# tengdj/lsbm

Hardware: AMD Instinct MI355X
Metric: CRC32C GiB/s over device-resident 4 KiB SSTable blocks (1 GPU); % HBM peak (higher is better)
Workload: dtype u8; 1 GPU; 1048576 x 4096 B device-resident blocks per GPU, batched crc32c::Value; blocks_per_gpu=1048576, block_bytes=4096, stride=4096, parallelism=1 independent shards, no data-path collective

## Files before the change

include/lsbm_crc32c.h:

```cpp
#ifndef LSBM_CRC32C_H_
#define LSBM_CRC32C_H_

#include <stddef.h>
#include <stdint.h>

#ifdef __cplusplus
extern "C" {
#endif

#define LSBM_OK 0
#define LSBM_ERR_INVALID (-1)
#define LSBM_ERR_NO_DEVICE (-2)
#define LSBM_ERR_HIP (-3)
#define LSBM_ERR_NOMEM (-4)
#define LSBM_ERR_CORRUPTION (-5)

#define LSBM_CRC32C_MASKED 0x1u

#define LSBM_CRC32C_MASK_DELTA 0xa282ead8u
#define LSBM_BLOCK_TRAILER_SIZE 5

uint32_t lsbm_crc32c_extend(uint32_t init_crc, const char* data, size_t n);
uint32_t lsbm_crc32c_value(const char* data, size_t n);
uint32_t lsbm_crc32c_mask(uint32_t crc);
uint32_t lsbm_crc32c_unmask(uint32_t masked_crc);

int lsbm_crc32c_init(int device);
int lsbm_crc32c_shutdown(void);
const char* lsbm_crc32c_version(void);
const char* lsbm_crc32c_last_error(void);

int lsbm_crc32c_fixed_dev(const void* d_base, uint64_t stride, uint64_t len, uint64_t n_blocks,
                          const uint32_t* d_init, uint32_t* d_out, uint32_t flags, void* stream);

int lsbm_crc32c_batch_dev(const void* d_base, const uint64_t* d_offsets, uint64_t n_blocks,
                          const uint32_t* d_init, uint32_t* d_out, uint32_t flags, void* stream);

int lsbm_crc32c_extents_dev(const void* d_base, const uint64_t* d_extents, uint64_t n_blocks,
// ... 16 lines not shown
int lsbm_log_crcs_dev(const uint8_t* d_log, uint64_t log_bytes, const uint64_t* d_headers,
                      uint64_t n_records, uint32_t* d_masked, uint32_t* d_nbad, void* stream);
int lsbm_log_verify_dev(const uint8_t* d_log, uint64_t log_bytes, const uint64_t* d_headers,
                        uint64_t n_records, uint8_t* d_ok, uint32_t* d_nbad, void* stream);

int lsbm_crc32c_batch_host(int device, const void* h_base, const uint64_t* h_offsets,
                           uint64_t n_blocks, const uint32_t* h_init, uint32_t* h_out,
                           uint32_t flags);

int lsbm_crc32c_batch_host_multi(const int* devices, int n_devices, const void* h_base,
                                 const uint64_t* h_offsets, uint64_t n_blocks,
                                 const uint32_t* h_init, uint32_t* h_out, uint32_t flags);

int lsbm_gather_dev(const void* d_src, const uint64_t* d_src_off, const uint64_t* d_len, uint64_t n,
                    void* d_dst, const uint64_t* d_dst_off, void* stream);

int lsbm_fill_splitmix64_dev(void* d_buf, uint64_t nbytes, uint64_t seed, void* stream);
int lsbm_stream_read_dev(const void* d_buf, uint64_t nbytes, uint32_t* d_sink, void* stream);

int lsbm_test_fail_host_pipeline(int chunks);
int lsbm_test_ragged_kernel(int which);

int lsbm_test_fixed_queue(int on);
int lsbm_test_sst_pieces(int on);

int lsbm_host_threads(void);

int lsbm_host_register(const void* p, uint64_t n);
int lsbm_host_unregister(const void* p);
unsigned long long lsbm_host_registered_bytes(void);
int lsbm_device_numa_node(int device);
int lsbm_test_pci_numa_node(const char* sysfs_root, const char* bus_id);
int lsbm_test_parse_cpulist(const char* list, int* cpus, int cap);
int lsbm_test_cgroup_quota(const char* cgroup_root);
int lsbm_test_pool_overlap(int callers, int jobs, int pieces, int piece_us, double* seconds);
int lsbm_test_cgroup_quota_of(const char* cgroup_root, const char* proc_cgroup);
int lsbm_test_pool_helpers(int pieces, int piece_us, int max_helpers);
int lsbm_test_locked_ranges(void);
long lsbm_test_locks_taken(void);
int lsbm_test_session_count(int device);
unsigned long long lsbm_test_pinned_bytes(int device);
int lsbm_test_pool_stress(int callers, int jobs, int max_pieces);
int lsbm_test_host_pinned(const void* p, size_t n);
int lsbm_test_zero_copy_max_mb(int mb);
int lsbm_test_host_copy(void* dst, const void* src, size_t n, int parallel);

// ... 6 lines not shown
```

lsbm_amd/_lib.py:

```python
import ctypes
import os

_HERE = os.path.dirname(os.path.abspath(__file__))
LIB_PATH = os.path.join(_HERE, "liblsbm_crc32c.so")
LIB_PATH = os.environ.get("LSBM_LIB_PATH") or LIB_PATH

LSBM_OK = 0
LSBM_ERR_INVALID = -1
LSBM_ERR_NO_DEVICE = -2
LSBM_ERR_HIP = -3
LSBM_ERR_NOMEM = -4
LSBM_ERR_CORRUPTION = -5
LSBM_CRC32C_MASKED = 0x1
LSBM_CRC32C_MASK_DELTA = 0xA282EAD8
LSBM_BLOCK_TRAILER_SIZE = 5

_u32, _u64, _int, _vp, _sz = (ctypes.c_uint32, ctypes.c_uint64, ctypes.c_int,
                              ctypes.c_void_p, ctypes.c_size_t)
SIGNATURES = {
    "lsbm_crc32c_extend": (_u32, [_u32, _vp, _sz]),
    "lsbm_crc32c_value": (_u32, [_vp, _sz]),
    "lsbm_crc32c_mask": (_u32, [_u32]),
    "lsbm_crc32c_unmask": (_u32, [_u32]),
    "lsbm_crc32c_init": (_int, [_int]),
    "lsbm_crc32c_shutdown": (_int, []),
    "lsbm_crc32c_version": (ctypes.c_char_p, []),
    "lsbm_crc32c_last_error": (ctypes.c_char_p, []),
    "lsbm_crc32c_fixed_dev": (_int, [_vp, _u64, _u64, _u64, _vp, _vp, _u32, _vp]),
    "lsbm_crc32c_batch_dev": (_int, [_vp, _vp, _u64, _vp, _vp, _u32, _vp]),
    "lsbm_crc32c_extents_dev": (_int, [_vp, _vp, _u64, _vp, _vp, _u32, _vp]),
    "lsbm_crc32c_verify_dev": (_int, [_vp, _vp, _u64, _vp, _vp, _vp, _vp, _u32, _vp]),
    "lsbm_sst_seal_dev": (_int, [_vp, _u64, _vp, _vp, _u64, _vp, _vp]),
    "lsbm_sst_verify_dev": (_int, [_vp, _u64, _vp, _u64, _vp, _vp, _vp]),
    "lsbm_sst_trailer_crcs_dev": (_int, [_vp, _u64, _vp, _vp, _u64, _vp, _vp, _vp]),
    "lsbm_log_seal_dev": (_int, [_vp, _u64, _vp, _u64, _vp, _vp, _vp]),
    "lsbm_log_verify_dev": (_int, [_vp, _u64, _vp, _u64, _vp, _vp, _vp]),
    "lsbm_log_crcs_dev": (_int, [_vp, _u64, _vp, _u64, _vp, _vp, _vp]),
    "lsbm_crc32c_batch_host": (_int, [_int, _vp, _vp, _u64, _vp, _vp, _u32]),
    "lsbm_crc32c_batch_host_multi": (_int, [_vp, _int, _vp, _vp, _u64, _vp, _vp, _u32]),
    "lsbm_gather_dev": (_int, [_vp, _vp, _vp, _u64, _vp, _vp, _vp]),
    "lsbm_fill_splitmix64_dev": (_int, [_vp, _u64, _u64, _vp]),
    "lsbm_stream_read_dev": (_int, [_vp, _u64, _vp, _vp]),
    "lsbm_test_fail_host_pipeline": (_int, [_int]),
    "lsbm_test_ragged_kernel": (_int, [_int]),
    "lsbm_test_fixed_queue": (_int, [_int]),
    "lsbm_test_sst_pieces": (_int, [_int]),
    "lsbm_host_threads": (_int, []),
    "lsbm_host_register": (_int, [ctypes.c_void_p, ctypes.c_uint64]),
    "lsbm_host_unregister": (_int, [ctypes.c_void_p]),
    "lsbm_host_registered_bytes": (ctypes.c_ulonglong, []),
    "lsbm_device_numa_node": (_int, [_int]),
    "lsbm_test_pci_numa_node": (_int, [ctypes.c_char_p, ctypes.c_char_p]),
    "lsbm_test_parse_cpulist": (_int, [ctypes.c_char_p, _vp, _int]),
    "lsbm_test_cgroup_quota": (_int, [ctypes.c_char_p]),
    "lsbm_test_cgroup_quota_of": (_int, [ctypes.c_char_p, ctypes.c_char_p]),
    "lsbm_test_pool_helpers": (_int, [_int, _int, _int]),
    "lsbm_test_locked_ranges": (_int, []),
    "lsbm_test_locks_taken": (ctypes.c_long, []),
    "lsbm_test_session_count": (_int, [_int]),
    "lsbm_test_pinned_bytes": (ctypes.c_ulonglong, [_int]),
    "lsbm_test_pool_overlap": (_int, [_int, _int, _int, _int, _vp]),
    "lsbm_test_host_pinned": (_int, [_vp, _sz]),
    "lsbm_test_host_copy": (_int, [_vp, _vp, _sz, _int]),
    "lsbm_test_pool_stress": (_int, [_int, _int, _int]),
    "lsbm_test_zero_copy_max_mb": (_int, [_int]),
    "lsbm_bloom_hash": (_u32, [_vp, _sz, _u32]),
    "lsbm_bloom_filter_bytes": (_u64, [_u64, _int]),
    "lsbm_bloom_k": (_u32, [_int]),
# ... 68 lines not shown
```

lsbm_amd/csrc/crc32c_engine.cc:

```cpp
#include <hip/hip_runtime_api.h>
#include <stdint.h>
#include <stdio.h>
#include <stdlib.h>
#include <string.h>

#include <algorithm>
#include <atomic>
#include <mutex>
#include <new>
#include <string>
#include <thread>
#include <vector>

#include "../../include/lsbm_crc32c.h"
#include "crc32c_types.h"
#include "engine_internal.h"
#include "gf2.h"
#include "host_numa.h"
#include "host_session.h"

namespace lsbm {

hipError_t launch_fixed(const uint8_t* base, uint64_t stride, uint32_t rows, uint64_t n_blocks,
                        const uint32_t* init, uint32_t* out, uint32_t flags, uint32_t k_value,
                        const DevConsts* dc, int grid, hipStream_t stream,
                        uint32_t* heads);
hipError_t launch_ragged(const RaggedArgs& a, int grid, hipStream_t stream);
bool ragged_uses_stream(const RaggedArgs& a);
int set_ragged_policy(int p);
hipError_t launch_range_bounds(const RaggedArgs& a, uint64_t P, uint32_t* bounds, int grid,
                               hipStream_t stream);
hipError_t launch_trailer_scatter(uint8_t* file, uint64_t limit, const uint64_t* handles, const uint8_t* types,
                                  const uint32_t* crcs, uint64_t n, int grid, hipStream_t stream);
hipError_t launch_fill(uint8_t* buf, uint64_t nbytes, uint64_t seed, int grid, hipStream_t stream);
hipError_t launch_gather(const uint8_t* src, const uint64_t* src_off, const uint64_t* len, uint64_t n,
                         uint8_t* dst, const uint64_t* dst_off, int grid, hipStream_t stream);
hipError_t launch_stream_read(const void* buf, uint64_t nbytes, uint32_t* sink, int grid,
                              hipStream_t stream);

namespace {

thread_local char t_last_error[256] = "";

int fail_hip(hipError_t e, const char* what) {
  snprintf(t_last_error, sizeof(t_last_error), "%s: %s", what, hipGetErrorString(e));
  return LSBM_ERR_HIP;
}
int fail(int code, const char* what) {
  snprintf(t_last_error, sizeof(t_last_error), "%s", what);
  return code;
}

constexpr int kMaxDevices = 64;

struct DeviceState {
  std::mutex mu;
  std::atomic<bool> ready{false};
  int status = LSBM_ERR_NO_DEVICE;
  DevConsts* d_consts = nullptr;
  int num_cus = 0;
};
DeviceState g_dev[kMaxDevices];

void build_consts(DevConsts* c) {
  gf2::byte_tables(gf2::byte_pow(kRowBytes), c->row_byte);
  {
    uint32_t tmp[1024];
    gf2::byte_tables(gf2::byte_pow(1), tmp);
    memcpy(c->t0, tmp, sizeof(c->t0));
  }
  gf2::Mat p = gf2::byte_pow(1);
  for (int k = 0; k < 64; k++) {
    gf2::nibble_tables(p, c->pow_nib[k]);
    p = gf2::mul(p, p);
  }
  const gf2::Mat inv1 = gf2::byte_pow(-1), fwd1 = gf2::byte_pow(1);
  {
    gf2::Mat m = gf2::identity();
    for (int z = 0; z < 128; z++, m = gf2::mul(inv1, m)) gf2::nibble_tables(m, c->neg_nib[z]);
  }
  gf2::nibble_tables(gf2::byte_pow(-4), c->neg4_nib);
  for (int li = 0; li < 8; li++) gf2::nibble_tables(gf2::byte_pow(116 - 16 * li), c->fin_nib[li]);
  memset(c->lds_image, 0, sizeof(c->lds_image));
#ifdef LSBM_LDS16
  {
// ... 68 lines not shown
  DevConsts* h = new (std::nothrow) DevConsts;
  if (!h) {
    st->status = fail(LSBM_ERR_NOMEM, "host alloc");
    hipSetDevice(prev);
    return;
  }
  build_consts(h);
  DevConsts* d = nullptr;
  e = hipMalloc(&d, sizeof(DevConsts));
  if (e == hipSuccess) e = hipMemcpy(d, h, sizeof(DevConsts), hipMemcpyHostToDevice);
  delete h;
  if (e != hipSuccess) {
    st->status = fail_hip(e, "device tables");
    if (d) hipFree(d);
    hipSetDevice(prev);
    return;
  }
  hipMemPool_t pool = nullptr;
  if (hipDeviceGetDefaultMemPool(&pool, dev) == hipSuccess && pool) {
    uint64_t keep = ~0ull;
    (void)hipMemPoolSetAttribute(pool, hipMemPoolAttrReleaseThreshold, &keep);
  }
  (void)hipGetLastError();
  st->d_consts = d;
  st->num_cus = cus;
  st->status = LSBM_OK;
  hipSetDevice(prev);
}

int ensure_device(int dev, DeviceState** out) {
  if (dev < 0 || dev >= kMaxDevices) return fail(LSBM_ERR_NO_DEVICE, "bad device ordinal");
  DeviceState* st = &g_dev[dev];
  if (!st->ready.load(std::memory_order_acquire)) {
    std::lock_guard<std::mutex> l(st->mu);
    if (!st->ready.load(std::memory_order_relaxed)) {
      init_device(dev, st);
      if (st->status != LSBM_OK) return st->status;
      st->ready.store(true, std::memory_order_release);
    }
  }
  *out = st;
  return LSBM_OK;
}

int current_device(DeviceState** out) {
  int dev = 0;
  hipError_t e = hipGetDevice(&dev);
  if (e != hipSuccess) return fail(LSBM_ERR_NO_DEVICE, "no current HIP device");
  return ensure_device(dev, out);
}

uint64_t fixed_split_blocks() {
  static const uint64_t b = [] {
    const char* v = getenv("LSBM_FIXED_SPLIT_BLOCKS");
    return v ? (uint64_t)strtoull(v, nullptr, 10) : (uint64_t)(1u << 20);
  }();
  return b;
}

std::atomic<int> g_fixed_queue{-1};
bool fixed_queue_on() {
  int q = g_fixed_queue.load(std::memory_order_relaxed);
  if (q < 0) {
    const char* v = getenv("LSBM_FIXED_QUEUE");
    q = (v && v[0] == '1') ? 1 : 0;
    int expect = -1;
    if (!g_fixed_queue.compare_exchange_strong(expect, q)) q = expect;
  }
  return q == 1;
}

std::atomic<int> g_sst_pieces{-1};
bool sst_pieces_on() {
  int q = g_sst_pieces.load(std::memory_order_relaxed);
  if (q < 0) {
    const char* v = getenv("LSBM_SST_PIECES");
    q = (v && v[0] == '1') ? 1 : 0;
    int expect = -1;
    if (!g_sst_pieces.compare_exchange_strong(expect, q)) q = expect;
  }
  return q == 1;
}

int grid_for(const DeviceState* st, uint64_t n_blocks) {
  const uint64_t groups = (n_blocks + 7) / 8;
  const uint64_t wgs = (groups + kWavesPerWg - 1) / kWavesPerWg;
  return (int)std::max<uint64_t>(1, std::min<uint64_t>(wgs, (uint64_t)st->num_cus));
}

uint32_t u_noinit() {
  static const uint32_t u = gf2::apply(gf2::byte_pow(-4), 0xffffffffu);
  return u;
// ... 56 lines not shown
  static const uint64_t per = [] {
    const char* v = getenv("LSBM_RAGGED_SPLIT_BLOCKS");
    return v ? (uint64_t)strtoull(v, nullptr, 10) : (uint64_t)0;
  }();
  if (!(per && a.mode == kModeOut && a.extents == kExtOffsets && a.n >= 2 * per))
    return run_ragged_one(a, stream);
  for (uint64_t f = 0; f < a.n;) {
    const uint64_t m = a.n - f >= 2 * per ? per : a.n - f;
    RaggedArgs b = a;
    b.offsets = a.offsets + f;
    b.n = m;
    b.out = a.out + f;
    if (a.init) b.init = a.init + f;
    const int rc = run_ragged_one(b, stream);
    if (rc != LSBM_OK) return rc;
    f += m;
  }
  return LSBM_OK;
}

}

extern "C" __attribute__((visibility("default"))) int lsbm_test_fixed_queue(int on) {
  if (on < -1 || on > 1) return -1;
  g_fixed_queue.store(on);
  return 0;
}

extern "C" __attribute__((visibility("default"))) int lsbm_test_sst_pieces(int on) {
  if (on < -1 || on > 1) return -1;
  g_sst_pieces.store(on);
  return 0;
}

int engine_fail(int code, const char* what) { return fail(code, what); }
int engine_fail_hip(hipError_t e, const char* what) { return fail_hip(e, what); }
int engine_current_cus(int* cus) {
  DeviceState* st = nullptr;
  const int rc = current_device(&st);
  if (rc == LSBM_OK) *cus = st->num_cus;
  return rc;
}

}

using namespace lsbm;

extern "C" {

// ... 6 lines not shown
}

__attribute__((visibility("default"))) int lsbm_crc32c_init(int device) {
  DeviceState* st = nullptr;
  return ensure_device(device, &st);
}

__attribute__((visibility("default"))) int lsbm_crc32c_shutdown(void) {
  HostSession::ShutdownAll();
  int prev = 0;
  const bool have_prev = hipGetDevice(&prev) == hipSuccess;
  int rc = LSBM_OK;
  for (int dev = 0; dev < kMaxDevices; dev++) {
    DeviceState* st = &g_dev[dev];
    std::lock_guard<std::mutex> l(st->mu);
    if (!st->ready.load()) continue;
    if (hipSetDevice(dev) != hipSuccess) {
      rc = fail(LSBM_ERR_HIP, "hipSetDevice");
      continue;
    }
    (void)hipDeviceSynchronize();
    if (st->d_consts) (void)hipFree(st->d_consts);
    st->d_consts = nullptr;
    st->status = LSBM_ERR_NO_DEVICE;
    st->ready.store(false);
  }
  if (have_prev) (void)hipSetDevice(prev);
  return rc;
}

__attribute__((visibility("default"))) int lsbm_crc32c_fixed_dev(
    const void* d_base, uint64_t stride, uint64_t len, uint64_t n_blocks, const uint32_t* d_init,
    uint32_t* d_out, uint32_t flags, void* stream) {
  if (n_blocks == 0) return LSBM_OK;
  if (!d_base || !d_out) return fail(LSBM_ERR_INVALID, "null pointer");
  if (flags & ~LSBM_CRC32C_MASKED) return fail(LSBM_ERR_INVALID, "unknown flags");
  DeviceState* st = nullptr;
  int rc = current_device(&st);
  if (rc != LSBM_OK) return rc;
  const uintptr_t b = reinterpret_cast<uintptr_t>(d_base);
  const bool fast = (b % 16 == 0) && (stride % 16 == 0) && len >= kRowBytes &&
                    (len % kRowBytes == 0) && stride >= len && stride <= (1ull << 28) &&
                    7 * stride + len < (1ull << 31) &&
                    n_blocks < (1ull << 34);
  if (fast) {
    const gf2::Mat an = gf2::byte_pow((int64_t)len);
    const uint32_t k_value = gf2::apply(an, 0xffffffffu) ^ 0xffffffffu;
    const uint64_t per = fixed_split_blocks();
    hipStream_t hs = static_cast<hipStream_t>(stream);
    uint64_t launches = 0, min_m = n_blocks;
    for (uint64_t f = 0; f < n_blocks; launches++) {
      const uint64_t m = (per && n_blocks - f >= 2 * per) ? per : n_blocks - f;
      min_m = std::min(min_m, m);
      f += m;
    }
    uint32_t* heads = nullptr;
    const uint64_t nwaves = (uint64_t)st->num_cus * kWavesPerWg;
    hipStreamCaptureStatus cap = hipStreamCaptureStatusNone;
    if (fixed_queue_on() && (min_m + 7) / 8 >= 4 * nwaves && hipStreamIsCapturing(hs, &cap) == hipSuccess &&
        cap == hipStreamCaptureStatusNone) {
      const size_t bytes = launches * kQueueWords * sizeof(uint32_t);
      if (hipMallocAsync(reinterpret_cast<void**>(&heads), bytes, hs) != hipSuccess) {
        (void)hipGetLastError();
        heads = nullptr;
      } else if (hipMemsetAsync(heads, 0, bytes, hs) != hipSuccess) {
        (void)hipGetLastError();
        (void)hipFreeAsync(heads, hs);
        heads = nullptr;
      }
    }
    hipError_t e = hipSuccess;
    uint64_t li = 0;
    for (uint64_t f = 0; f < n_blocks && e == hipSuccess; li++) {
      const uint64_t m = (per && n_blocks - f >= 2 * per) ? per : n_blocks - f;
      e = launch_fixed(static_cast<const uint8_t*>(d_base) + f * stride, stride,
                       (uint32_t)(len / kRowBytes), m, d_init ? d_init + f : nullptr, d_out + f, flags,
                       k_value, st->d_consts, grid_for(st, m), hs, heads ? heads + li * kQueueWords : nullptr);
      f += m;
    }
    if (heads) (void)hipFreeAsync(heads, hs);
    return e == hipSuccess ? LSBM_OK : fail_hip(e, "crc32c_fixed_kernel");
  }
  RaggedArgs a = {};
  a.base = static_cast<const uint8_t*>(d_base);
  a.stride = stride;
  a.len = len;
  a.extents = kExtFixed;
  a.n = n_blocks;
  a.init = d_init;
  a.out = d_out;
  a.flags = flags;
  a.mode = kModeOut;
  return run_ragged(a, static_cast<hipStream_t>(stream));
}

__attribute__((visibility("default"))) int lsbm_crc32c_batch_dev(
    const void* d_base, const uint64_t* d_offsets, uint64_t n_blocks, const uint32_t* d_init,
    uint32_t* d_out, uint32_t flags, void* stream) {
  if (n_blocks == 0) return LSBM_OK;
  if (!d_base || !d_offsets || !d_out) return fail(LSBM_ERR_INVALID, "null pointer");
// ... 452 lines not shown
```

lsbm_amd/csrc/crc32c_kernels.hip:

```cpp
#include <hip/hip_runtime.h>
#include <stdint.h>
#include <stdlib.h>

#include <atomic>

#include "crc32c_units.h"

namespace lsbm {


#ifdef LSBM_DIAG_STAMPS
extern "C" __attribute__((visibility("default"))) int lsbm_diag_stamps(uint64_t* host, int n) {
  (void)n;
  return hipMemcpyFromSymbol(host, HIP_SYMBOL(g_stamps), sizeof(uint64_t) * 4 * 65536) == hipSuccess ? 0 : -1;
}
#endif
#define DIAG_STAMP(k) DIAG_STAMP_W(k, wave)

#ifndef LSBM_PF
#define LSBM_PF 4
#endif
constexpr uint32_t kPF = LSBM_PF;


// ... 2 lines not shown
#define LOAD_BANK(X, r0)                                                          \
  do {                                                                            \
    _Pragma("unroll") for (uint32_t k_ = 0; k_ < kPF; k_++) {                     \
      const uint32_t rr_ = (r0) + k_ < rows ? (r0) + k_ : rows - 1;               \
      X[k_] = __builtin_bit_cast(                                                 \
          u32x4, __builtin_amdgcn_raw_buffer_load_b128(rsrc, loff + rr_ * kRowBytes, 0, \
                                                       kAuxNT));                  \
    }                                                                             \
  } while (0)


#define ABSORB(X, r0)                                                       \
  do {                                                                      \
    _Pragma("unroll") for (uint32_t k_ = 0; k_ < kPF; k_++) {               \
      if ((r0) + k_ < rows) STEP_ROW(X[k_]);                                \
    }                                                                       \
  } while (0)

template <bool kHasInit, uint32_t kRows>
__global__ __launch_bounds__(kBlockThreads) void crc32c_fixed_kernel(
    const uint8_t* __restrict__ base, uint64_t stride, uint32_t rows_arg, uint64_t n_blocks,
    const uint32_t* __restrict__ init, uint32_t* __restrict__ out, uint32_t flags,
    uint32_t k_value ,
    const DevConsts* __restrict__ dc, uint32_t* __restrict__ heads ) {
  const uint32_t rows = kRows ? kRows : rows_arg;
  const uint32_t lane = threadIdx.x & 63u;
  const uint32_t g = lane >> 3, li = lane & 7u;
  const uint32_t lb = row_lane_base(lane);
  const uint32_t L0 = lb | kRowTab[0], L1 = lb | kRowTab[1], L2 = lb | kRowTab[2], L3 = lb | kRowTab[3];
  const uint32_t lane_fin = kNibFin | lb;
  const uint32_t wave_in_wg = __builtin_amdgcn_readfirstlane(threadIdx.x >> 6);
  const uint64_t wave = (uint64_t)blockIdx.x * kWavesPerWg + wave_in_wg;
  const uint64_t nwaves = (uint64_t)gridDim.x * kWavesPerWg;
  const uint64_t ngroups = (n_blocks + 7) / 8;

  u32x4 a[kPF], b[kPF];
  __amdgpu_buffer_rsrc_t rsrc;
  uint32_t loff;
  auto set_group = [&](uint64_t grp) {
    const uint64_t blk = grp * 8 + g;
    const uint64_t nb = n_blocks - grp * 8 < 8 ? n_blocks - grp * 8 : 8;
    rsrc = __builtin_amdgcn_make_buffer_rsrc(const_cast<uint8_t*>(base + grp * 8 * stride),
                                             (short)0, (int)((nb - 1) * stride + rows * kRowBytes),
                                             0x00020000);
    loff = (blk < n_blocks ? g : 0u) * (uint32_t)stride + 16u * li;
    asm volatile("" : "+v"(loff));
  };
#ifndef LSBM_WG_STATIC
  __shared__ uint32_t s_next;
  if (threadIdx.x == 0) s_next = kWavesPerWg;
  auto next_grp = [&](uint64_t) -> uint64_t {
    uint32_t k = 0;
    if (lane == 0) k = atomicAdd(&s_next, 1u);
    k = __builtin_amdgcn_readfirstlane(k);
#ifdef LSBM_WG_ROTATE
    const uint64_t c = k / kWavesPerWg;
    return c * nwaves + (((uint64_t)blockIdx.x + c) % gridDim.x) * kWavesPerWg + (k % kWavesPerWg);
#else
    return (uint64_t)(k / kWavesPerWg) * nwaves + (uint64_t)blockIdx.x * kWavesPerWg + (k % kWavesPerWg);
#endif
  };
#else
  auto next_grp = [&](uint64_t gp) -> uint64_t { return gp + nwaves; };
#endif
  __shared__ uint32_t s_wq[kWqWords];
  const WgQueue<kWavesPerWg> wq{heads, (lds_u32*)s_wq,
                                ngroups > nwaves ? (ngroups - nwaves + kWavesPerWg - 1) / kWavesPerWg : 0};
  if (heads && threadIdx.x == 0) wq.init(xcc_id());

  uint64_t grp = wave;
  DIAG_STAMP(0);
  bool loaded = false;
  if (grp < ngroups) {
    set_group(grp);
    LOAD_BANK(a, 0);
    if (kRows == 0 || kPF < rows) LOAD_BANK(b, kPF);
    loaded = true;
  }
  load_lds_tables(g_lds, dc);
  DIAG_STAMP(1);

  uint32_t pend_pub = heads && wave_in_wg == 0 ? kWqLead : 0u;
  for (;;) {
    if (grp < ngroups) {
      const uint64_t blk = grp * 8 + g;
      const bool valid = blk < n_blocks;
      if (!loaded) {
        set_group(grp);
        LOAD_BANK(a, 0);
        if (kRows == 0 || kPF < rows) LOAD_BANK(b, kPF);
      }
      loaded = false;
      if (pend_pub) {
        wq.publish(pend_pub);
        pend_pub = 0;
      }
      uint32_t c0 = a[0].x, c1 = a[0].y, c2 = a[0].z, c3 = a[0].w;
#pragma unroll
      for (uint32_t k = 1; k < kPF; k++)
        if (k < rows) STEP_ROW(a[k]);
      uint32_t r = kPF;
      while (r < rows) {
        if (kRows == 0 || r + kPF < rows) LOAD_BANK(a, r + kPF);
        ABSORB(b, r);
        r += kPF;
// ... 5 lines not shown
#ifdef LSBM_ABL_NO_MERGE
      const uint32_t raw = c0 ^ c1 ^ c2 ^ c3;
#else
      const uint32_t raw = merge_braids(g_lds, c0, c1, c2, c3, lane_fin);
#endif
      if (li == 7u && valid) {
        uint32_t crc;
        if (kHasInit)
          crc = raw ^ advance_glb(dc, init[blk] ^ 0xffffffffu, (uint64_t)rows * kRowBytes) ^
                0xffffffffu;
        else
          crc = raw ^ k_value;
        out[blk] = (flags & 1u) ? mask_crc(crc) : crc;
      }
    } else if (pend_pub) {
      wq.publish(pend_pub);
      pend_pub = 0;
    }
    if (!heads) {
      grp = next_grp(grp);
      if (grp >= ngroups) break;
      continue;
    }
    const uint32_t k = wq.take(), bt = k / kWavesPerWg, slot = k % kWavesPerWg;
    if (slot == 0) pend_pub = bt + kWqLead;
    const uint32_t it = wq.read(bt);
    if (it == kWqNone) {
      if (pend_pub) wq.publish(pend_pub);
      break;
    }
    grp = nwaves + (uint64_t)it * kWavesPerWg + slot;
  }
  DIAG_STAMP(2);
  DIAG_XCC_W(wave);
}

__device__ __forceinline__ void cas_merge(unsigned long long* p, uint64_t m, uint64_t v) {
  unsigned long long old = *p;
  for (;;) {
    const unsigned long long want = (old & ~m) | (v & m);
    if (want == old) return;
    const unsigned long long got = atomicCAS(p, old, want);
    if (got == old) return;
    old = got;
  }
}

__device__ __forceinline__ void merge_bytes(uint64_t img, uint64_t limit, uint64_t t, uint32_t nb, uint64_t v) {
  const uint32_t sh = (uint32_t)(t & 7u);
  const uint64_t w0a = t & ~7ull;
  const bool two = sh + nb > 8;
  if (w0a < img || w0a + (two ? 16u : 8u) > img + limit) {
    uint8_t* tb = reinterpret_cast<uint8_t*>(t);
    for (uint32_t k = 0; k < nb; k++) tb[k] = (uint8_t)(v >> (8 * k));
    return;
// ... 118 lines not shown
    const uint32_t loff = g * 4096u + 16u * li;
#pragma unroll
    for (uint32_t r0 = 0; r0 < 32; r0 += 4) {
      u32x4 v[4];
#pragma unroll
      for (uint32_t k = 0; k < 4; k++)
        v[k] = __builtin_bit_cast(u32x4, __builtin_amdgcn_raw_buffer_load_b128(
                                             rsrc, loff + (r0 + k) * kRowBytes, 0, kAuxNT));
#pragma unroll
      for (uint32_t k = 0; k < 4; k++) acc ^= xor3(v[k].x, v[k].y, v[k].z) ^ v[k].w;
    }
  }
  const uint64_t tail0 = ngroups * 32768;
  for (uint64_t i = tail0 + ((uint64_t)blockIdx.x * blockDim.x + threadIdx.x) * 16; i + 16 <= nbytes;
       i += (uint64_t)gridDim.x * blockDim.x * 16) {
    const u32x4 v = *reinterpret_cast<const u32x4*>(base + i);
    acc ^= v.x ^ v.y ^ v.z ^ v.w;
  }
  if (acc == 0x9e3779b9u) sink[blockIdx.x & 1023u] = acc;
}

hipError_t launch_fixed(const uint8_t* base, uint64_t stride, uint32_t rows, uint64_t n_blocks,
                        const uint32_t* init, uint32_t* out, uint32_t flags, uint32_t k_value,
                        const DevConsts* dc, int grid, hipStream_t stream, uint32_t* heads) {
#define LSBM_LAUNCH_FIXED(HI, R)                                                        \
  hipLaunchKernelGGL((crc32c_fixed_kernel<HI, R>), dim3(grid), dim3(kBlockThreads), 0, stream, \
                     base, stride, rows, n_blocks, init, out, flags, k_value, dc, heads)
  if (init) {
    if (rows == 32) LSBM_LAUNCH_FIXED(true, 32);
    else if (rows == 512) LSBM_LAUNCH_FIXED(true, 512);
    else LSBM_LAUNCH_FIXED(true, 0);
  } else {
    if (rows == 32) LSBM_LAUNCH_FIXED(false, 32);
    else if (rows == 512) LSBM_LAUNCH_FIXED(false, 512);
    else LSBM_LAUNCH_FIXED(false, 0);
  }
#undef LSBM_LAUNCH_FIXED
  return hipGetLastError();
}

hipError_t launch_range_bounds(const RaggedArgs& a, uint64_t P, uint32_t* bounds, int grid,
                               hipStream_t stream) {
  const uint64_t want = (P / 2 + 1 + 3) / 4;
  const dim3 g((unsigned)(want < (uint64_t)grid ? want : grid));
  if (a.extents == kExtOffsets)
    hipLaunchKernelGGL(range_bounds_kernel<kExtOffsets>, g, dim3(256), 0, stream, a, P, bounds);
  else if (a.extents == kExtHandles)
    hipLaunchKernelGGL(range_bounds_kernel<kExtHandles>, g, dim3(256), 0, stream, a, P, bounds);
  else
    return hipErrorInvalidValue;
// ... 109 lines not shown
```

lsbm_amd/csrc/crc32c_types.h:

```cpp
#pragma once
#include <stdint.h>

#if (defined(LSBM_DIAG_NO_STORE) || defined(LSBM_DIAG_VERIFY_WRITEBACK) || \
     defined(LSBM_DIAG_NO_PROBE_WRITES)) && !defined(LSBM_DIAG_BUILD)
#error "LSBM_DIAG_* result-changing macros need LSBM_DIAG_BUILD (A/B variant builds only)"
#endif

namespace lsbm {

constexpr int kRowBytes = 128;
constexpr int kGroupLanes = 8;
constexpr int kWaveLanes = 64;
constexpr int kBlockThreads = 1024;
constexpr int kWavesPerWg = kBlockThreads / kWaveLanes;
constexpr int kStreamThreads = 1024;
constexpr int kStreamWavesPerWg = kStreamThreads / kWaveLanes;
constexpr uint32_t kLdsByteTabBytes = 131072;
constexpr uint32_t kNibA4 = 0x20000;
constexpr uint32_t kNibA8 = kNibA4 + 512;
constexpr uint32_t kNibA12 = kNibA4 + 1024;
#ifdef LSBM_LDS16
constexpr uint32_t kByteA4 = 0x10000;
#endif
constexpr uint32_t kNibFin = 0x20800;
constexpr uint32_t kRowPowTables = 21;
constexpr uint32_t kNibRowPow = kNibFin + 8 * 16 * 32 * 4;
constexpr uint32_t kRowPowLo = 9;
constexpr uint32_t kNibPow2 = kNibRowPow;
constexpr uint32_t kNibNeg128 = kNibRowPow + 8 * 512;
constexpr uint32_t kNibNeg4 = kNibRowPow + kRowPowTables * 512;
constexpr uint32_t kStreamHM = kNibNeg4 + 512;
constexpr uint32_t kStreamMasks = 17 * 18 / 2;
constexpr uint32_t km_entry(uint32_t lo, uint32_t hi) {
  return hi >= 16u ? lo : 17u + 16u * lo - ((lo * (lo - 1u)) >> 1) + hi - lo;
}
constexpr uint32_t kStreamR0 = kStreamHM + kStreamMasks * 16;
constexpr uint32_t kLdsBytes = kStreamR0 + 128 * 4;
constexpr uint32_t kLdsWords = kLdsBytes / 4;
constexpr uint32_t kLdsKernelWords = 20;

#ifndef LSBM_QUEUE_STRIDE
#define LSBM_QUEUE_STRIDE 16
#endif
constexpr uint32_t kQueueHeads = 8;
constexpr uint32_t kQueueStride = LSBM_QUEUE_STRIDE;
constexpr uint32_t kQueueWords = kQueueHeads * kQueueStride;
static_assert(kLdsBytes % 16 == 0 && kLdsBytes + 4u * kLdsKernelWords <= 160u * 1024u,
              "one LDS image per CU, plus the kernels' work counters");
static_assert(kStreamHM % 16 == 0, "ds_read_b128 of a mask");

constexpr uint32_t kShiftCols = 512;
constexpr uint32_t kFinCols = 129;

struct DevConsts {
  uint32_t row_byte[4 * 256];
  uint32_t t0[256];
  uint32_t pow_nib[64][128];
  uint32_t neg_nib[128][128];
  uint32_t neg4_nib[128];
  uint32_t fin_nib[8][128];
  alignas(16) uint32_t shift_cols[kShiftCols][32];
  alignas(16) uint32_t fin_cols[kFinCols][32];
  alignas(16) uint32_t lds_image[kLdsWords];
  alignas(16) uint32_t zero16[4];
};

enum ExtentKind : uint32_t {
  kExtOffsets = 0,
  kExtHandles = 1,
// ... 54 lines not shown
```

lsbm_amd/csrc/crc32c_units.h:

```cpp
#pragma once
#include <hip/hip_runtime.h>
#include <stdint.h>

#include "crc32c_device.h"

namespace lsbm {

__shared__ uint32_t g_lds[kLdsWords];


__device__ __forceinline__ uint32_t xcc_id() {
  uint32_t x;
  asm volatile("s_getreg_b32 %0, hwreg(HW_REG_XCC_ID, 0, 4)" : "=s"(x));
  return x & (kQueueHeads - 1);
}

__device__ __forceinline__ uint32_t queue_take(uint32_t* heads, uint32_t h) {
  uint32_t j = 0;
  if ((threadIdx.x & 63u) == 0) j = atomicAdd(heads + h * kQueueStride, 1u);
  return __builtin_amdgcn_readfirstlane(j);
}

constexpr uint32_t kWqRing = 4, kWqLead = 1, kWqNone = 0xffffffffu, kSpinCap = 1u << 20;
constexpr uint32_t kWqWords = 3 + 3 * kWqRing;
static_assert(kWqLead == 1, "wave 0 publishes batch 1 only: the batches before the first slot-0 taker's");
static_assert(kWqRing > kWqLead, "an entry is reused only after its batch's slots were all taken");

typedef __attribute__((address_space(3))) uint32_t lds_u32;

template <uint32_t W>
struct WgQueue {
  uint32_t* heads;
  lds_u32* s;
  uint64_t items;

  __device__ __forceinline__ volatile lds_u32* v(uint32_t i) const { return (volatile lds_u32*)(s + i); }
  __device__ __forceinline__ void init(uint32_t xcc) const {
    *v(0) = W;
    *v(1) = xcc;
    *v(2) = 0;
    for (uint32_t e = 0; e < kWqRing; e++) {
      *v(3 + e) = 0;
      *v(3 + kWqRing + e) = kWqNone;
      *v(3 + 2 * kWqRing + e) = 0;
    }
  }
  __device__ __forceinline__ uint32_t take() const {
    uint32_t k = 0;
    if ((threadIdx.x & 63u) == 0) k = __atomic_fetch_add(s, 1u, __ATOMIC_RELAXED);
    return __builtin_amdgcn_readfirstlane(k);
  }
  __device__ __forceinline__ uint32_t rd(uint32_t i) const { return __builtin_amdgcn_readfirstlane(*v(i)); }
  __device__ __forceinline__ void publish(uint32_t x) const {
    const uint32_t e = x % kWqRing, pe = (x - 1) % kWqRing;
    uint32_t spins = 0;
    if (x >= 2)
      while (rd(3 + pe) != x - 1 && ++spins < kSpinCap) __builtin_amdgcn_s_sleep(2);
    if (x > kWqRing)
      while (rd(3 + 2 * kWqRing + e) != W && ++spins < kSpinCap) __builtin_amdgcn_s_sleep(2);
    uint32_t h = rd(1), out = rd(2), it = kWqNone;
    while (spins < kSpinCap && out < kQueueHeads) {
      const uint64_t cand = (uint64_t)queue_take(heads, h) * kQueueHeads + h;
      if (cand < items) {
        it = (uint32_t)cand;
        break;
      }
      if (++out < kQueueHeads) h = (h + 1) & (kQueueHeads - 1);
    }
    if ((threadIdx.x & 63u) == 0) {
      *v(1) = h;
      *v(2) = out;
      *v(3 + kWqRing + e) = it;
      *v(3 + 2 * kWqRing + e) = 0;
      *v(3 + e) = x;
    }
  }
  __device__ __forceinline__ uint32_t read(uint32_t b) const {
    const uint32_t e = b % kWqRing;
    uint32_t spins = 0;
    while (rd(3 + e) != b)
      if (++spins >= kSpinCap) return kWqNone;
      else __builtin_amdgcn_s_sleep(2);
    const uint32_t it = rd(3 + kWqRing + e);
    if ((threadIdx.x & 63u) == 0) __atomic_fetch_add(s + 3 + 2 * kWqRing + e, 1u, __ATOMIC_RELAXED);
    return it;
  }
};

#ifdef LSBM_DIAG_STAMPS
static __device__ uint64_t g_stamps[4][65536];
#define DIAG_STAMP_W(k, w)                                                          \
  do {                                                                              \
    if ((threadIdx.x & 63u) == 0) g_stamps[k][(w) & 65535] = __builtin_amdgcn_s_memrealtime(); \
  } while (0)
#define DIAG_XCC_W(w)                                                               \
  do {                                                                              \
    if ((threadIdx.x & 63u) == 0) {                                                 \
      uint32_t xcc_;                                                                \
      asm volatile("s_getreg_b32 %0, hwreg(HW_REG_XCC_ID, 0, 4)" : "=s"(xcc_));     \
      g_stamps[3][(w) & 65535] = xcc_;                                              \
    }                                                                               \
  } while (0)
#else
#define DIAG_STAMP_W(k, w) do { } while (0)
#define DIAG_XCC_W(w) do { } while (0)
// ... 744 lines not shown
```

Baseline: 6343 GiB/s.

## Enable fixed-kernel work queue by default with static prefix and pooled heads

Turns the cross-XCC dynamic work queue for the fixed-stride CRC kernel on by default in a new mode 2. Each wave statically owns most of its rows and only the final tail fraction of row groups is balanced through the queue. Queue head counters now come from a preallocated device pool that the last workgroup resets in-kernel, replacing a per-call hipMallocAsync plus memset. The queue stride is widened so heads sit further apart, and a pinned host fault word records spin-cap hits. This aims to cut tail imbalance across XCDs and remove per-call allocation overhead, at the cost of extra atomics, pool bookkeeping and new failure paths.

```diff
diff --git a/include/lsbm_crc32c.h b/include/lsbm_crc32c.h
--- a/include/lsbm_crc32c.h
+++ b/include/lsbm_crc32c.h
@@ -14,6 +14,7 @@
 #define LSBM_ERR_HIP (-3)
 #define LSBM_ERR_NOMEM (-4)
 #define LSBM_ERR_CORRUPTION (-5)
+#define LSBM_ERR_QUEUE_FAULT (-6)
 
 #define LSBM_CRC32C_MASKED 0x1u
 
@@ -76,6 +77,10 @@
 int lsbm_test_ragged_kernel(int which);
 
 int lsbm_test_fixed_queue(int on);
+int lsbm_test_fixed_tail(int min_rows, int tail_rows);
+int lsbm_test_queue_fault(int device, int value);
+int lsbm_test_queue_pool(int on);
+int lsbm_test_queue_pool_busy(int device);
 int lsbm_test_sst_pieces(int on);
 
 int lsbm_host_threads(void);
diff --git a/lsbm_amd/_lib.py b/lsbm_amd/_lib.py
--- a/lsbm_amd/_lib.py
+++ b/lsbm_amd/_lib.py
@@ -11,6 +11,7 @@
 LSBM_ERR_HIP = -3
 LSBM_ERR_NOMEM = -4
 LSBM_ERR_CORRUPTION = -5
+LSBM_ERR_QUEUE_FAULT = -6
 LSBM_CRC32C_MASKED = 0x1
 LSBM_CRC32C_MASK_DELTA = 0xA282EAD8
 LSBM_BLOCK_TRAILER_SIZE = 5
@@ -44,6 +45,10 @@
     "lsbm_test_fail_host_pipeline": (_int, [_int]),
     "lsbm_test_ragged_kernel": (_int, [_int]),
     "lsbm_test_fixed_queue": (_int, [_int]),
+    "lsbm_test_fixed_tail": (_int, [_int, _int]),
+    "lsbm_test_queue_fault": (_int, [_int, _int]),
+    "lsbm_test_queue_pool": (_int, [_int]),
+    "lsbm_test_queue_pool_busy": (_int, [_int]),
     "lsbm_test_sst_pieces": (_int, [_int]),
     "lsbm_host_threads": (_int, []),
     "lsbm_host_register": (_int, [ctypes.c_void_p, ctypes.c_uint64]),
diff --git a/lsbm_amd/csrc/crc32c_engine.cc b/lsbm_amd/csrc/crc32c_engine.cc
--- a/lsbm_amd/csrc/crc32c_engine.cc
+++ b/lsbm_amd/csrc/crc32c_engine.cc
@@ -24,7 +24,7 @@
 hipError_t launch_fixed(const uint8_t* base, uint64_t stride, uint32_t rows, uint64_t n_blocks,
                         const uint32_t* init, uint32_t* out, uint32_t flags, uint32_t k_value,
                         const DevConsts* dc, int grid, hipStream_t stream,
-                        uint32_t* heads);
+                        uint32_t* heads, uint32_t own_rows, uint32_t* fault, uint32_t* done, uint32_t* busy);
 hipError_t launch_ragged(const RaggedArgs& a, int grid, hipStream_t stream);
 bool ragged_uses_stream(const RaggedArgs& a);
 int set_ragged_policy(int p);
@@ -59,8 +59,22 @@
   int status = LSBM_ERR_NO_DEVICE;
   DevConsts* d_consts = nullptr;
   int num_cus = 0;
+  uint32_t cap_local = 0;
+  uint32_t* cap_word = &cap_local;
+  std::mutex pool_mu;
+  uint32_t* pool = nullptr;
+  uint32_t* pool_busy = nullptr;
+  uint32_t pool_cursor = 0;
 };
+constexpr uint32_t kPoolRegions = 8;
+constexpr uint32_t kPoolSets = kPoolRegions * kQueueSetsPerRegion;
+constexpr uint32_t kPoolWords = kPoolRegions * kQueueWords + kPoolSets * kQueueDoneStride;
+constexpr uint32_t kPinnedBusyAt = 16;
 DeviceState g_dev[kMaxDevices];
+
+bool queue_faulted(const DeviceState* st) {
+  return __atomic_load_n(st->cap_word, __ATOMIC_RELAXED) != 0;
+}
 
 void build_consts(DevConsts* c) {
   gf2::byte_tables(gf2::byte_pow(kRowBytes), c->row_byte);
@@ -175,6 +189,26 @@
     (void)hipMemPoolSetAttribute(pool, hipMemPoolAttrReleaseThreshold, &keep);
   }
   (void)hipGetLastError();
+  uint32_t* w = nullptr;
+  e = hipHostMalloc(reinterpret_cast<void**>(&w), (kPinnedBusyAt + kPoolSets) * sizeof(uint32_t), hipHostMallocDefault);
+  if (e != hipSuccess || !w) {
+    st->status = fail_hip(e, "queue fault word");
+    hipFree(d);
+    hipSetDevice(prev);
+    return;
+  }
+  memset(w, 0, (kPinnedBusyAt + kPoolSets) * sizeof(uint32_t));
+  *w = st->cap_local;
+  st->cap_word = w;
+  uint32_t* hpool = nullptr;
+  if (hipMalloc(reinterpret_cast<void**>(&hpool), kPoolWords * sizeof(uint32_t)) == hipSuccess &&
+      hipMemset(hpool, 0, kPoolWords * sizeof(uint32_t)) == hipSuccess) {
+    st->pool = hpool;
+    st->pool_busy = w + kPinnedBusyAt;
+  } else {
+    if (hpool) (void)hipFree(hpool);
+    (void)hipGetLastError();
+  }
   st->d_consts = d;
   st->num_cus = cus;
   st->status = LSBM_OK;
@@ -184,14 +218,17 @@
 int ensure_device(int dev, DeviceState** out) {
   if (dev < 0 || dev >= kMaxDevices) return fail(LSBM_ERR_NO_DEVICE, "bad device ordinal");
   DeviceState* st = &g_dev[dev];
+  const char* const faulted = "the cross-XCC queue hit its spin cap on this device: results were lost";
   if (!st->ready.load(std::memory_order_acquire)) {
     std::lock_guard<std::mutex> l(st->mu);
     if (!st->ready.load(std::memory_order_relaxed)) {
+      if (queue_faulted(st)) return fail(LSBM_ERR_QUEUE_FAULT, faulted);
       init_device(dev, st);
       if (st->status != LSBM_OK) return st->status;
       st->ready.store(true, std::memory_order_release);
     }
   }
+  if (queue_faulted(st)) return fail(LSBM_ERR_QUEUE_FAULT, faulted);
   *out = st;
   return LSBM_OK;
 }
@@ -211,16 +248,57 @@
   return b;
 }
 
+constexpr int kFixedQueueDefault = 2;
+constexpr uint32_t kFullQueueMinRows = 4;
+constexpr uint32_t kTailMinRows = 8;
+constexpr uint32_t kTailSixteenths = 2;
 std::atomic<int> g_fixed_queue{-1};
-bool fixed_queue_on() {
+std::atomic<int> g_tail_min_rows{-1}, g_tail_rows{-1};
+int fixed_queue_mode() {
   int q = g_fixed_queue.load(std::memory_order_relaxed);
   if (q < 0) {
     const char* v = getenv("LSBM_FIXED_QUEUE");
-    q = (v && v[0] == '1') ? 1 : 0;
+    q = (v && v[0] >= '0' && v[0] <= '2' && v[1] == 0) ? v[0] - '0' : kFixedQueueDefault;
     int expect = -1;
     if (!g_fixed_queue.compare_exchange_strong(expect, q)) q = expect;
   }
-  return q == 1;
+  return q;
+}
+
+std::atomic<int> g_queue_pool{1};
+int take_head_set(DeviceState* st) {
+  if (!st->pool || !g_queue_pool.load(std::memory_order_relaxed)) return -1;
+  std::lock_guard<std::mutex> l(st->pool_mu);
+  for (uint32_t i = 0; i < kPoolSets; i++) {
+    const uint32_t s = (st->pool_cursor + i) % kPoolSets;
+    if (__atomic_load_n(st->pool_busy + s, __ATOMIC_ACQUIRE) == 0) {
+      __atomic_store_n(st->pool_busy + s, 1u, __ATOMIC_RELAXED);
+      st->pool_cursor = s + 1;
+      return (int)s;
+    }
+  }
+  return -1;
+}
+void release_head_set(DeviceState* st, int s) {
+  __atomic_store_n(st->pool_busy + s, 0u, __ATOMIC_RELEASE);
+}
+uint32_t* set_heads(const DeviceState* st, int s) {
+  return st->pool + (size_t)(s / kQueueSetsPerRegion) * kQueueWords + (size_t)(s % kQueueSetsPerRegion) * 32u;
+}
+uint32_t* set_done(const DeviceState* st, int s) {
+  return st->pool + (size_t)kPoolRegions * kQueueWords + (size_t)s * kQueueDoneStride;
+}
+
+uint32_t fixed_own_rows(int mode, uint64_t ngroups, uint64_t nwaves) {
+  const uint64_t rows = (ngroups + nwaves - 1) / nwaves;
+  if (mode == 1) return ngroups >= kFullQueueMinRows * nwaves ? 1u : 0u;
+  if (mode != 2) return 0;
+  const int hook_min = g_tail_min_rows.load(std::memory_order_relaxed);
+  const int hook_tail = g_tail_rows.load(std::memory_order_relaxed);
+  const uint64_t min_rows = hook_min > 0 ? (uint64_t)hook_min : kTailMinRows;
+  if (ngroups < min_rows * nwaves || rows > 0xffffffull) return 0;
+  const uint64_t tail = hook_tail > 0 ? (uint64_t)hook_tail : std::max<uint64_t>(1, rows * kTailSixteenths / 16);
+  return (uint32_t)(rows > tail ? rows - tail : 1);
 }
 
 std::atomic<int> g_sst_pieces{-1};
@@ -323,9 +401,39 @@
 }
 
 extern "C" __attribute__((visibility("default"))) int lsbm_test_fixed_queue(int on) {
-  if (on < -1 || on > 1) return -1;
+  if (on < -1 || on > 2) return -1;
   g_fixed_queue.store(on);
   return 0;
+}
+
+extern "C" __attribute__((visibility("default"))) int lsbm_test_fixed_tail(int min_rows, int tail_rows) {
+  if (min_rows < -1 || min_rows == 0 || tail_rows < -1 || tail_rows == 0) return -1;
+  g_tail_min_rows.store(min_rows);
+  g_tail_rows.store(tail_rows);
+  return 0;
+}
+
+extern "C" __attribute__((visibility("default"))) int lsbm_test_queue_pool(int on) {
+  if (on < 0 || on > 1) return -1;
+  g_queue_pool.store(on);
+  return 0;
+}
+
+extern "C" __attribute__((visibility("default"))) int lsbm_test_queue_pool_busy(int device) {
+  if (device < 0 || device >= kMaxDevices) return -1;
+  DeviceState* st = &g_dev[device];
+  if (!st->ready.load(std::memory_order_acquire) || !st->pool) return -1;
+  std::lock_guard<std::mutex> l(st->pool_mu);
+  int busy = 0;
+  for (uint32_t i = 0; i < kPoolSets; i++) busy += __atomic_load_n(st->pool_busy + i, __ATOMIC_ACQUIRE) != 0;
+  return busy;
+}
+
+extern "C" __attribute__((visibility("default"))) int lsbm_test_queue_fault(int device, int value) {
+  if (device < 0 || device >= kMaxDevices || value < 0 || value > 1) return -1;
+  DeviceState* st = &g_dev[device];
+  std::lock_guard<std::mutex> l(st->mu);
+  return (int)__atomic_exchange_n(st->cap_word, (uint32_t)value, __ATOMIC_RELAXED);
 }
 
 extern "C" __attribute__((visibility("default"))) int lsbm_test_sst_pieces(int on) {
@@ -378,6 +486,14 @@
     (void)hipDeviceSynchronize();
     if (st->d_consts) (void)hipFree(st->d_consts);
     st->d_consts = nullptr;
+    if (st->pool) (void)hipFree(st->pool);
+    st->pool = nullptr;
+    st->pool_busy = nullptr;
+    if (st->cap_word != &st->cap_local) {
+      st->cap_local = *st->cap_word;
+      (void)hipHostFree(st->cap_word);
+      st->cap_word = &st->cap_local;
+    }
     st->status = LSBM_ERR_NO_DEVICE;
     st->ready.store(false);
   }
@@ -413,25 +529,42 @@
     uint32_t* heads = nullptr;
     const uint64_t nwaves = (uint64_t)st->num_cus * kWavesPerWg;
     hipStreamCaptureStatus cap = hipStreamCaptureStatusNone;
-    if (fixed_queue_on() && (min_m + 7) / 8 >= 4 * nwaves && hipStreamIsCapturing(hs, &cap) == hipSuccess &&
+    const int qmode = fixed_queue_mode();
+    std::vector<int> sets;
+    if (fixed_own_rows(qmode, (min_m + 7) / 8, nwaves) != 0 && hipStreamIsCapturing(hs, &cap) == hipSuccess &&
         cap == hipStreamCaptureStatusNone) {
-      const size_t bytes = launches * kQueueWords * sizeof(uint32_t);
-      if (hipMallocAsync(reinterpret_cast<void**>(&heads), bytes, hs) != hipSuccess) {
-        (void)hipGetLastError();
-        heads = nullptr;
-      } else if (hipMemsetAsync(heads, 0, bytes, hs) != hipSuccess) {
-        (void)hipGetLastError();
-        (void)hipFreeAsync(heads, hs);
-        heads = nullptr;
+      for (uint64_t i = 0; i < launches; i++) {
+        const int sidx = take_head_set(st);
+        if (sidx < 0) break;
+        sets.push_back(sidx);
+      }
+      if (sets.size() != launches) {
+        for (int sidx : sets) release_head_set(st, sidx);
+        sets.clear();
+        const size_t bytes = launches * kQueueWords * sizeof(uint32_t);
+        if (hipMallocAsync(reinterpret_cast<void**>(&heads), bytes, hs) != hipSuccess) {
+          (void)hipGetLastError();
+          heads = nullptr;
+        } else if (hipMemsetAsync(heads, 0, bytes, hs) != hipSuccess) {
+          (void)hipGetLastError();
+          (void)hipFreeAsync(heads, hs);
+          heads = nullptr;
+        }
       }
     }
     hipError_t e = hipSuccess;
     uint64_t li = 0;
     for (uint64_t f = 0; f < n_blocks && e == hipSuccess; li++) {
       const uint64_t m = (per && n_blocks - f >= 2 * per) ? per : n_blocks - f;
+      const bool pooled = !sets.empty();
+      uint32_t* const h = pooled ? set_heads(st, sets[li]) : heads ? heads + li * kQueueWords : nullptr;
       e = launch_fixed(static_cast<const uint8_t*>(d_base) + f * stride, stride,
                        (uint32_t)(len / kRowBytes), m, d_init ? d_init + f : nullptr, d_out + f, flags,
-                       k_value, st->d_consts, grid_for(st, m), hs, heads ? heads + li * kQueueWords : nullptr);
+                       k_value, st->d_consts, grid_for(st, m), hs, h,
+                       h ? fixed_own_rows(qmode, (m + 7) / 8, nwaves) : 1u, st->cap_word,
+                       pooled ? set_done(st, sets[li]) : nullptr, pooled ? st->pool_busy + sets[li] : nullptr);
+      if (e != hipSuccess && pooled)
+        for (uint64_t k = li; k < launches; k++) release_head_set(st, sets[k]);
       f += m;
     }
     if (heads) (void)hipFreeAsync(heads, hs);
diff --git a/lsbm_amd/csrc/crc32c_kernels.hip b/lsbm_amd/csrc/crc32c_kernels.hip
--- a/lsbm_amd/csrc/crc32c_kernels.hip
+++ b/lsbm_amd/csrc/crc32c_kernels.hip
@@ -48,7 +48,10 @@
     const uint8_t* __restrict__ base, uint64_t stride, uint32_t rows_arg, uint64_t n_blocks,
     const uint32_t* __restrict__ init, uint32_t* __restrict__ out, uint32_t flags,
     uint32_t k_value ,
-    const DevConsts* __restrict__ dc, uint32_t* __restrict__ heads ) {
+    const DevConsts* __restrict__ dc, uint32_t* __restrict__ heads ,
+    uint32_t own_rows ,
+    uint32_t* __restrict__ fault ,
+    uint32_t* __restrict__ done, uint32_t* __restrict__ busy ) {
   const uint32_t rows = kRows ? kRows : rows_arg;
   const uint32_t lane = threadIdx.x & 63u;
   const uint32_t g = lane >> 3, li = lane & 7u;
@@ -90,8 +93,10 @@
   auto next_grp = [&](uint64_t gp) -> uint64_t { return gp + nwaves; };
 #endif
   __shared__ uint32_t s_wq[kWqWords];
+  const uint64_t own_groups = (uint64_t)own_rows * nwaves;
   const WgQueue<kWavesPerWg> wq{heads, (lds_u32*)s_wq,
-                                ngroups > nwaves ? (ngroups - nwaves + kWavesPerWg - 1) / kWavesPerWg : 0};
+                                ngroups > own_groups ? (ngroups - own_groups + kWavesPerWg - 1) / kWavesPerWg : 0,
+                                own_rows, fault};
   if (heads && threadIdx.x == 0) wq.init(xcc_id());
 
   uint64_t grp = wave;
@@ -106,7 +111,7 @@
   load_lds_tables(g_lds, dc);
   DIAG_STAMP(1);
 
-  uint32_t pend_pub = heads && wave_in_wg == 0 ? kWqLead : 0u;
+  uint32_t pend_pub = heads && wave_in_wg == 0 && own_rows == 1 ? kWqLead : 0u;
   for (;;) {
     if (grp < ngroups) {
       const uint64_t blk = grp * 8 + g;
@@ -158,15 +163,22 @@
       if (grp >= ngroups) break;
       continue;
     }
-    const uint32_t k = wq.take(), bt = k / kWavesPerWg, slot = k % kWavesPerWg;
+    const uint32_t k = wq.take(), slot = k % kWavesPerWg;
+    if (k < own_rows * kWavesPerWg) {
+      if (k == (own_rows - 1) * kWavesPerWg) pend_pub = kWqLead;
+      grp = (uint64_t)(k / kWavesPerWg) * nwaves + (uint64_t)blockIdx.x * kWavesPerWg + slot;
+      continue;
+    }
+    const uint32_t bt = k / kWavesPerWg - own_rows + 1;
     if (slot == 0) pend_pub = bt + kWqLead;
     const uint32_t it = wq.read(bt);
     if (it == kWqNone) {
       if (pend_pub) wq.publish(pend_pub);
       break;
     }
-    grp = nwaves + (uint64_t)it * kWavesPerWg + slot;
-  }
+    grp = own_groups + (uint64_t)it * kWavesPerWg + slot;
+  }
+  if (heads) wq.leave(done, busy);
   DIAG_STAMP(2);
   DIAG_XCC_W(wave);
 }
@@ -331,10 +343,11 @@
 
 hipError_t launch_fixed(const uint8_t* base, uint64_t stride, uint32_t rows, uint64_t n_blocks,
                         const uint32_t* init, uint32_t* out, uint32_t flags, uint32_t k_value,
-                        const DevConsts* dc, int grid, hipStream_t stream, uint32_t* heads) {
+                        const DevConsts* dc, int grid, hipStream_t stream, uint32_t* heads, uint32_t own_rows,
+                        uint32_t* fault, uint32_t* done, uint32_t* busy) {
 #define LSBM_LAUNCH_FIXED(HI, R)                                                        \
   hipLaunchKernelGGL((crc32c_fixed_kernel<HI, R>), dim3(grid), dim3(kBlockThreads), 0, stream, \
-                     base, stride, rows, n_blocks, init, out, flags, k_value, dc, heads)
+                     base, stride, rows, n_blocks, init, out, flags, k_value, dc, heads, own_rows, fault, done, busy)
   if (init) {
     if (rows == 32) LSBM_LAUNCH_FIXED(true, 32);
     else if (rows == 512) LSBM_LAUNCH_FIXED(true, 512);
diff --git a/lsbm_amd/csrc/crc32c_types.h b/lsbm_amd/csrc/crc32c_types.h
--- a/lsbm_amd/csrc/crc32c_types.h
+++ b/lsbm_amd/csrc/crc32c_types.h
@@ -40,11 +40,13 @@
 constexpr uint32_t kLdsKernelWords = 20;
 
 #ifndef LSBM_QUEUE_STRIDE
-#define LSBM_QUEUE_STRIDE 16
+#define LSBM_QUEUE_STRIDE 1040
 #endif
 constexpr uint32_t kQueueHeads = 8;
 constexpr uint32_t kQueueStride = LSBM_QUEUE_STRIDE;
 constexpr uint32_t kQueueWords = kQueueHeads * kQueueStride;
+constexpr uint32_t kQueueSetsPerRegion = kQueueStride >= 64 ? kQueueStride / 32 : 1;
+constexpr uint32_t kQueueDoneStride = 32;
 static_assert(kLdsBytes % 16 == 0 && kLdsBytes + 4u * kLdsKernelWords <= 160u * 1024u,
               "one LDS image per CU, plus the kernels' work counters");
 static_assert(kStreamHM % 16 == 0, "ds_read_b128 of a mask");
diff --git a/lsbm_amd/csrc/crc32c_units.h b/lsbm_amd/csrc/crc32c_units.h
--- a/lsbm_amd/csrc/crc32c_units.h
+++ b/lsbm_amd/csrc/crc32c_units.h
@@ -22,7 +22,7 @@
 }
 
 constexpr uint32_t kWqRing = 4, kWqLead = 1, kWqNone = 0xffffffffu, kSpinCap = 1u << 20;
-constexpr uint32_t kWqWords = 3 + 3 * kWqRing;
+constexpr uint32_t kWqWords = 4 + 3 * kWqRing;
 static_assert(kWqLead == 1, "wave 0 publishes batch 1 only: the batches before the first slot-0 taker's");
 static_assert(kWqRing > kWqLead, "an entry is reused only after its batch's slots were all taken");
 
@@ -33,12 +33,15 @@
   uint32_t* heads;
   lds_u32* s;
   uint64_t items;
+  uint32_t own_rows;
+  uint32_t* fault;
 
   __device__ __forceinline__ volatile lds_u32* v(uint32_t i) const { return (volatile lds_u32*)(s + i); }
   __device__ __forceinline__ void init(uint32_t xcc) const {
     *v(0) = W;
     *v(1) = xcc;
     *v(2) = 0;
+    *v(3 + 3 * kWqRing) = 0;
     for (uint32_t e = 0; e < kWqRing; e++) {
       *v(3 + e) = 0;
       *v(3 + kWqRing + e) = kWqNone;
@@ -51,6 +54,10 @@
     return __builtin_amdgcn_readfirstlane(k);
   }
   __device__ __forceinline__ uint32_t rd(uint32_t i) const { return __builtin_amdgcn_readfirstlane(*v(i)); }
+  __device__ __forceinline__ void cap_hit() const {
+    if ((threadIdx.x & 63u) == 0 && fault)
+      __hip_atomic_store(fault, 1u, __ATOMIC_RELAXED, __HIP_MEMORY_SCOPE_SYSTEM);
+  }
   __device__ __forceinline__ void publish(uint32_t x) const {
     const uint32_t e = x % kWqRing, pe = (x - 1) % kWqRing;
     uint32_t spins = 0;
@@ -67,6 +74,7 @@
       }
       if (++out < kQueueHeads) h = (h + 1) & (kQueueHeads - 1);
     }
+    if (spins >= kSpinCap) cap_hit();
     if ((threadIdx.x & 63u) == 0) {
       *v(1) = h;
       *v(2) = out;
@@ -75,12 +83,25 @@
       *v(3 + e) = x;
     }
   }
+  __device__ __forceinline__ void leave(uint32_t* done, uint32_t* busy) const {
+    if (!done || (threadIdx.x & 63u) != 0) return;
+    if (__atomic_fetch_add(s + 3 + 3 * kWqRing, 1u, __ATOMIC_RELAXED) != W - 1) return;
+    if (__hip_atomic_fetch_add(done, 1u, __ATOMIC_RELAXED, __HIP_MEMORY_SCOPE_AGENT) != gridDim.x - 1) return;
+    for (uint32_t h = 0; h < kQueueHeads; h++)
+      __hip_atomic_store(heads + h * kQueueStride, 0u, __ATOMIC_RELAXED, __HIP_MEMORY_SCOPE_AGENT);
+    __hip_atomic_store(done, 0u, __ATOMIC_RELAXED, __HIP_MEMORY_SCOPE_AGENT);
+    __hip_atomic_store(busy, 0u, __ATOMIC_RELEASE, __HIP_MEMORY_SCOPE_SYSTEM);
+  }
   __device__ __forceinline__ uint32_t read(uint32_t b) const {
     const uint32_t e = b % kWqRing;
     uint32_t spins = 0;
     while (rd(3 + e) != b)
-      if (++spins >= kSpinCap) return kWqNone;
-      else __builtin_amdgcn_s_sleep(2);
+      if (++spins >= kSpinCap) {
+        cap_hit();
+        return kWqNone;
+      } else {
+        __builtin_amdgcn_s_sleep(2);
+      }
     const uint32_t it = rd(3 + kWqRing + e);
     if ((threadIdx.x & 63u) == 0) __atomic_fetch_add(s + 3 + 2 * kWqRing + e, 1u, __ATOMIC_RELAXED);
     return it;
```

After: 6473 GiB/s, median of 6. +2.0%, better.
